# cloudflare/flow-pipeline

Measured on AMD Instinct MI355X. Metric: FlowMessages/sec aggregated into flows_5m, higher is better.
Workload: dtype u64

## Files before the change

flow-pipeline_amd/csrc/ingest.cuh:

```cuda
#pragma once
#include <hip/hip_runtime.h>
#include <stdint.h>

#include "sinks.cuh"

#ifndef FA_FOLD_EVERY
#define FA_FOLD_EVERY 4
#endif
#ifndef FA_LT_KEEP
#define FA_LT_KEEP 8u
#endif
namespace fa {

struct NoHook {
    __device__ __forceinline__ void operator()() const {}
};
struct LaneTally {
    uint32_t ok = 0, direct = 0, second = 0, misfit8 = 0, late = 0;
    uint32_t tick = 0;
};
template <int MODE, uint32_t KEYSETS, uint32_t COLS, bool T8 = false, int CANDM = -1, class Hook = NoHook>
__device__ __forceinline__ void lane_work(const KArgs& a, LdsTable<LDS_SLOTS>& lt, LdsMinutes& lm, uint32_t* part_cnt, const uint32_t* tile,
                                          bool mine, uint32_t pos, uint32_t end, uint32_t rec_idx, uint32_t tb_base,
                                          LaneTally& tally, uint32_t& pmode, uint32_t& lt_seen, uint32_t& lt_hits,
                                          uint4* bins, uint32_t* bin_cnt, uint32_t& fill_out, Hook&& after_parse = Hook(),
                                          CmsLds* cl = nullptr, uint32_t* cms_scratch = nullptr, HotAddrs* hot = nullptr,
                                          uint32_t* wpart_cnt = nullptr, uint32_t* seq = nullptr) {
    constexpr uint32_t TB = bin_cap<T8, bin_line(KEYSETS)>();
    bool sure = false, framed_ok = false;
    Rec r;
    rec_clear(r);
    if (mine) {
        LdsSrc src{tile};
        framed_ok = true;
        if (a.framed && !(FA_DBG(a, DBG_NO_FRAME))) {
            uint32_t pl = 0;
            const uint32_t i = pos >> 2;
            framed_ok = frame_short(fa_alignbyte(src.dw(i + 1), src.dw(i), pos), end - pos, pl);
            pos += pl;
        }
        sure = framed_ok && (FA_DBG(a, DBG_NO_PARSE)) != 0;
    }
    if (!FA_DBG(a, DBG_NO_PARSE)) {
        LdsAbsSrc src;
        const uint32_t tile_at = (uint32_t)(uintptr_t)(const __attribute__((address_space(3))) uint32_t*)tile;
        pos += tile_at;
        end += tile_at;
        const uint32_t n_mine = (uint32_t)__builtin_popcountll(__builtin_amdgcn_ballot_w64(framed_ok));
        auto most = [&](bool c) { return 2u * (uint32_t)__builtin_popcountll(__builtin_amdgcn_ballot_w64(c)) > n_mine; };
        if (pmode == 0u && !FA_DBG(a, DBG_LOOP_PARSER)) {
            if (framed_ok) sure = parse_tmpl<COLS, SHAPE_MOCKER>(src, pos, end, r);
        }
        bool need = framed_ok && !sure;
        if (pmode <= 1u && FA_ANY(need) && !FA_DBG(a, DBG_LOOP_PARSER | DBG_NO_SECOND)) {
            if (need) {
                rec_clear(r);
                sure = parse_tmpl<COLS, SHAPE_GOFLOW>(src, pos, end, r);
            }
            if (pmode < 1u && most(need && sure)) pmode = 1u;
        }
        need = framed_ok && !sure;
        if (pmode <= 2u && FA_ANY(need) && !FA_DBG(a, DBG_LOOP_PARSER | DBG_NO_SECOND)) {
            if (need) {
                rec_clear(r);
                sure = parse_canon<COLS, true>(src, pos, end, r);
            }
            if (pmode < 2u && most(need && sure)) pmode = 2u;
        }
        if (pmode == 4u && seq != nullptr && !FA_DBG(a, DBG_NO_SECOND)) {
            if (framed_ok) {
                sure = parse_seq<COLS>(src, pos, end, r, seq + 2, fa_uniform(seq[0]));
                if (!FA_DBG(a, DBG_LOOP_PARSER)) tally.second += sure ? 1u : 0u;
            }
        }
// ... 75 lines not shown
            if (vd && keys_on) pd = keyset_probe(a, a.ks_dst, dh1);
        }
    }
    if (ks_on<KEYSETS>(a, FA_KEYS_AS_PAIR)) {
        uint64_t k0 = 0, k1 = 0;
        const bool lt_on = lt_seen != 0xffffffffu && !(FA_DBG(a, DBG_NO_LDS_TABLE));
        uint32_t h = 0;
        if (!T8 || lt_on) {
            pack_key(tb, r.src_as, r.dst_as, r.etype, k0, k1);
            h = key_hash(k0, k1);
        }
        const uint64_t b = r.bytes, p = r.packets, c = 1;
        bool pending = sure;
        if (lt_on) {
            if (pending) pending = !lds_table_add<LDS_SLOTS, LDS_PROBES>(lt, k0, k1, h, b, p, c);
            lt_seen += (uint32_t)__builtin_popcountll(__builtin_amdgcn_ballot_w64(sure));
            lt_hits += (uint32_t)__builtin_popcountll(__builtin_amdgcn_ballot_w64(sure && !pending));
            if (lt_seen >= 256u) {
                if (lt_hits * FA_LT_KEEP < lt_seen) lt_seen = 0xffffffffu;
                else lt_seen = lt_hits = 0;
            }
        }
        uint32_t fill_part = 0xffffffffu;
        bool fits = false;
        uint32_t part = 0;
        uint4 tv = make_uint4(0, 0, 0, 0);
        if (pending && a.seg) {
            const uint32_t tbr = tb - tb_base;
            if (T8) {
                fits = t8_fits(r.src_as, r.dst_as, tbr, b, p, r.etype);
                const uint2 tc = t8_pack(r.src_as, r.dst_as, (uint32_t)b, (uint32_t)p, tbr, r.etype, tb_base, part);
                tv.x = tc.x;
                tv.y = tc.y;
                if (FA_ANY(!fits)) tally.misfit8 += (!fits && tup16_fits(tbr, b, p, r.etype)) ? 1u : 0u;
            } else {
                fits = tup16_fits(tbr, b, p, r.etype);
                part = h >> (32 - a.plog2);
                tv = tup16_pack(r.src_as, r.dst_as, (uint32_t)b, (uint32_t)p, tbr, r.etype);
            }
        }
        if (bins) {
            auto claim = [&]() {
                const uint32_t slot = __hip_atomic_fetch_add(&bin_cnt[part], 1u, __ATOMIC_ACQUIRE, __HIP_MEMORY_SCOPE_WORKGROUP) & 0xffffu;
                if (slot < TB) {
                    if (T8) reinterpret_cast<uint2*>(bins)[part * TB + slot] = make_uint2(tv.x, tv.y);
                    else bins[part * TB + slot] = tv;
                    __hip_atomic_fetch_add(&bin_cnt[part], 0x10000u, __ATOMIC_RELEASE, __HIP_MEMORY_SCOPE_WORKGROUP);
                    fill_part = slot == TB - 1 ? part : fill_part;
                    pending = false;
                }
            };
            if (pending && fits) {
                claim();
                if (pending) {
                    const uint32_t ob = lds_add_rtn_u32(&part_cnt[part], 0x10000u) >> 16;
                    if (ob < a.capb) {
                        const size_t at = (size_t)part * a.region + (size_t)blockIdx.x * a.capq + (a.capq - 1u - ob);
                        if (FA_DBG(a, DBG_TUPLE_LOCAL)) {
                            reinterpret_cast<uint2*>(a.seg)[(size_t)blockIdx.x * 512u + (at & 511u)] = make_uint2(tv.x, tv.y);
                        } else if (!(FA_DBG(a, DBG_NO_TUPLE_STORE | DBG_NO_SINGLES))) {
                            if (T8) reinterpret_cast<uint2*>(a.seg)[at] = make_uint2(tv.x, tv.y);
                            else a.seg[at] = tv;
                        }
                        pending = false;
                    } else {
                        lds_add_u32(&part_cnt[part], 0xffff0000u);
                    }
                }
            }
        }
        fill_out = fill_part;
        if (__builtin_amdgcn_ballot_w64(pending) != 0ull && !(FA_DBG(a, DBG_NO_GLOBAL))) {
            Slot* sp = nullptr;
            const KArgs ca = cold_args();
            if (pending) {
                tally.direct++;
                if (T8 && !lt_on) {
                    pack_key(tb, r.src_as, r.dst_as, r.etype, k0, k1);
                    h = key_hash(k0, k1);
                }
                sp = table_find_or_claim(ca, k0, k1, h);
                if (!sp) spill_park(ca, k0, k1, b, p, c);
            }
            quad_atomic_update(sp, b, p, c);
        }
    }
    if (KEYSETS & (FA_KEYS_SRCADDR_CMS | FA_KEYS_DSTADDR_CMS)) {
        if (!(FA_DBG(a, DBG_NO_CMS))) {
            if (cl && (CANDM >= 0 || a.cseg)) {
                uint32_t* list = const_cast<uint32_t*>(tile) + 256;
                if (on_s) cms_scatter(a, *cl, list, 0u, vs, ws, sh1, sh2);
                if (on_d) cms_scatter(a, *cl, list, 1u, vd, wd, dh1, dh2);
            } else {
                if (vs) cms_add(a.cms_src, a.cms_depth, a.cms_wl2, a.cms_seed, r.src, ws, a.cms_nrep);
                if (vd) cms_add(a.cms_dst, a.cms_depth, a.cms_wl2, a.cms_seed, r.dst, wd, a.cms_nrep);
            }
        }
        if (keys_on && !cand) keyset_finish2(a, vs, ps, sh1, slo, shi, vd, pd, dh1, dlo, dhi);
        if (keys_on && cand) {
            const bool is = vs && cand_pass(a.cand_src, a.cms_depth, a.cms_wl2, cms_key(sh1, sh2, a.cms_wl2), cw0s);
            const bool id = vd && cand_pass(a.cand_dst, a.cms_depth, a.cms_wl2, cms_key(dh1, dh2, a.cms_wl2), cw0d);
            if (FA_ANY(is || id) && !FA_DBG(a, DBG_CAND_NO_SET)) {
                if (is) keyset_insert_h(a, a.ks_src, slo, shi, sh1);
                if (id) keyset_insert_h(a, a.ks_dst, dlo, dhi, dh1);
            }
        }
// ... 204 lines not shown
            for (int i0 = 0; i0 < LDS_SLOTS; i0 += BLOCK) {
                const int i = i0 + tid;
                Slot* sp = nullptr;
                unsigned long long b = 0, p = 0, c = 0;
                if (i < LDS_SLOTS) {
                    const unsigned long long k0 = lt.k0[i], k1 = lt.k1[i];
                    b = lt.bytes[i];
                    p = lt.packets[i];
                    c = lt.count[i];
                    if (k0 != 0 && k1 != 0 && c != 0) {
                        sp = table_find_or_claim(a, k0, k1, key_hash(k0, k1));
                        if (!sp) spill_park(a, k0, k1, b, p, c);
                    }
                }
                quad_atomic_update(sp, b, p, c);
            }
        }
        block_counters_add(ctr_scratch, a.ctr, tally);
    }
}

template <bool ON>
struct CmsLdsOpt {
    CmsLds v;
    __device__ __forceinline__ CmsLds* get() { return &v; }
};
template <>
struct CmsLdsOpt<false> {
    __device__ __forceinline__ CmsLds* get() { return nullptr; }
};
template <uint32_t KEYSETS>
constexpr int wtile_block() { return wt_lean(KEYSETS) ? WBLOCK : WBLOCK_CMS; }
template <uint32_t KEYSETS>
constexpr int wtile_stride() { return wt_stride(KEYSETS); }
template <bool ON>
struct HotAddrsOpt {
    HotAddrs v;
    __device__ __forceinline__ HotAddrs* get() { return &v; }
};
template <>
struct HotAddrsOpt<false> {
    __device__ __forceinline__ HotAddrs* get() { return nullptr; }
};

template <uint32_t KEYSETS, bool T8, bool SEQ = false, int CANDM = -1>
__global__ __launch_bounds__(wtile_block<KEYSETS>(), wt_lean(KEYSETS) ? 6 : 4) void wtile_kernel(KArgs a) {
    constexpr uint32_t BL = bin_line(KEYSETS);
    constexpr uint32_t TB = bin_cap<T8, BL>();
    constexpr uint32_t COLS = cols_for_keysets<KEYSETS>();
    constexpr int WBLOCK = wtile_block<KEYSETS>();
    constexpr bool HAS_CMS = (KEYSETS & (FA_KEYS_SRCADDR_CMS | FA_KEYS_DSTADDR_CMS)) != 0;
    constexpr int WAVES = WBLOCK / 64;
    constexpr int WT_STRIDE = wtile_stride<KEYSETS>();
    __shared__ CmsLdsOpt<HAS_CMS> cms_lds;
    __shared__ HotAddrsOpt<HAS_CMS> hot_lds;
    __shared__ uint32_t cms_scratch_all[HAS_CMS ? WAVES * 16 : 1];
    __shared__ __attribute__((aligned(16))) uint32_t tiles[WAVES * WT_STRIDE / 4];
    __shared__ __attribute__((aligned(16))) uint4 bins[NPART_MAX * BL];
    __shared__ uint32_t bin_cnt[NPART_MAX];
    __shared__ uint32_t part_cnt[NPART_MAX];
    __shared__ uint32_t flush_scratch[WAVES * 16];
    constexpr bool HAS_APP = (KEYSETS & FA_KEYS_ADDR_PORT_PROTO) != 0;
    __shared__ uint32_t wpart_cnt[HAS_APP ? (1u << WIDE_PLOG2_MAX) + 2u : 1u];
    __shared__ LdsTable<LDS_SLOTS> lt;
    __shared__ LdsMinutes lm;
    constexpr bool HAS_SEQ = SEQ && KEYSETS == FA_KEYS_AS_PAIR;
    static_assert(!SEQ || KEYSETS == FA_KEYS_AS_PAIR, "the learnt-order variant exists for the flows_5m rollup alone");
    __shared__ uint32_t seq_all[HAS_SEQ ? WAVES * (SEQ_MAX + 2) : 1];

    const uint32_t tid = threadIdx.x, lane = tid & 63;
    const uint32_t wave = __builtin_amdgcn_readfirstlane(tid >> 6);
    if (HAS_SEQ && lane < 2) seq_all[wave * (SEQ_MAX + 2) + lane] = 0;
    if (KEYSETS & FA_KEYS_AS_PAIR) {
        lds_table_clear(lt);
        for (int i = tid; i < NPART_MAX; i += WBLOCK) {
            part_cnt[i] = 0;
            bin_cnt[i] = 0;
        }
    }
    if (KEYSETS & FA_KEYS_MINUTE_SERIES) lds_minutes_clear(lm);
    if (HAS_APP)
        for (int i = tid; i < (1 << WIDE_PLOG2_MAX) + 2; i += WBLOCK) wpart_cnt[i] = i < (1 << WIDE_PLOG2_MAX) ? 0u : 0xffffffffu;
    CmsLds* const cl = (HAS_CMS && (CANDM >= 0 || a.cseg)) ? cms_lds.get() : nullptr;
    HotAddrs* const hot = (HAS_CMS && (KEYSETS != KS_ALL || (a.key_sets & (FA_KEYS_SRCADDR_CMS | FA_KEYS_DSTADDR_CMS)))) ? hot_lds.get() : nullptr;
    if (HAS_CMS && cl)
        for (int i = tid; i < (int)(CMS_SETS * CMS_NPART); i += WBLOCK) {
            cl->bin_cnt[i] = 0;
            cl->part_cnt[i] = 0;
        }
    if (HAS_CMS && hot)
        for (int i = tid; i < (int)(CMS_SETS * HOT_SLOTS); i += WBLOCK) {
            const int set = i / HOT_SLOTS, sl = i % HOT_SLOTS;
            const size_t at = (size_t)blockIdx.x * (CMS_SETS * HOT_SLOTS) + i;
            const uint32_t tg = a.hot_seed_tag ? a.hot_seed_tag[at] : 0u;
            if (tg >= 2u) {
                const HotSeed sd = a.hot_seed[at];
                hot->lo[set][sl] = sd.lo;
                hot->hi[set][sl] = sd.hi;
                hot->w[set][sl] = 0;
            }
            hot->touched[set][sl] = 0;
            *hot->tag(set, sl) = tg >= 2u ? tg : 0u;
        }
    uint32_t* tile = tiles + wave * (WT_STRIDE / 4);

    LaneTally tally;
    uint32_t lt_seen = 0, lt_hits = 0, pmode = 0;
    uint32_t tb_base = 0;
    const uint32_t ntiles = (a.n + a.tile_recs - 1) / a.tile_recs;
    __shared__ uint32_t next_k;
    if (tid == 0) next_k = 2u * WAVES;
    const uint32_t wg_pos = (gridDim.x & 7u) == 0u ? (blockIdx.x & 7u) * (gridDim.x >> 3) + (blockIdx.x >> 3) : blockIdx.x;
    auto tile_after_next = [&]() {
        uint32_t k = 0;
        if (lane == 0) k = lds_add_rtn_u32(&next_k, 1u);
        return (uint32_t)__builtin_amdgcn_readfirstlane((int)k) * gridDim.x + wg_pos;
    };
    struct __attribute__((packed, aligned(4))) OffPair {
        uint32_t lo, hi;
    };
    struct Tile {
        uint32_t r0, nrec;
        uint32_t q0, q1;
    };
    auto tile_load = [&](uint32_t t) {
        Tile d{0, 0, 0, 0};
        if (t < ntiles) {
            d.r0 = t * a.tile_recs;
            d.nrec = min(a.tile_recs, a.n - d.r0);
            if (lane < d.nrec) {
                const OffPair v = *reinterpret_cast<const OffPair*>(a.off + d.r0 + lane);
                d.q0 = v.lo;
                d.q1 = v.hi;
            }
        }
        return d;
    };
    constexpr uint32_t CAP = (uint32_t)WT_STRIDE - 16u;
    auto issue_dma = [&](uint32_t lo, uint32_t hi) {
        const uint32_t cbase = lo & ~15u;
        const uint32_t nbytes = hi > cbase ? min(hi - cbase, CAP) : 0u;
        for (uint32_t o = lane * 16u; o < nbytes; o += 1024u)
            __builtin_amdgcn_global_load_lds((const __attribute__((address_space(1))) void*)(a.buf + cbase + o),
                                             (__attribute__((address_space(3))) void*)(tile + (o - lane * 16u) / 4u), 16, 0, 2);
    };
    Tile cur = tile_load(wave * gridDim.x + wg_pos);
    uint32_t cur_lo = (uint32_t)__builtin_amdgcn_readfirstlane((int)cur.q0);
    uint32_t cur_hi = cur.nrec ? min((uint32_t)__builtin_amdgcn_readlane((int)cur.q1, (int)(cur.nrec - 1u)), a.len) : 0u;
    bool live = lane < cur.nrec;
    __syncthreads();
    issue_dma(cur_lo, cur_hi);
    Tile nxt = tile_load((wave + WAVES) * gridDim.x + wg_pos);
    tb_base = probe_tb_base(a);
    if (blockIdx.x == 0 && tid == 0) a.ctr->tb_base = tb_base;
    uint32_t t2 = 0;
    bool t2_have = false;
    while (cur.nrec != 0) {
        dma_wait_all();
        if (!t2_have) {
            t2 = tile_after_next();
            t2_have = true;
        }
        const uint32_t cbase = cur_lo & ~15u;
        const bool valid = live && cur.q1 >= cur.q0 && cur.q0 >= cur_lo && cur.q1 <= cur_hi;
        const bool staged = valid && cur.q1 - cbase <= CAP;
        bool rest = valid && !staged;
        const bool hopeless = (live && !valid) || (rest && cur.q0 == cur_lo);
        if (FA_ANY(hopeless)) {
            if (hopeless) {
                unsigned int j = atomicAdd(&a.ctr->exotic_count[a.par], 1u);
                a.exotic_idx[j] = cur.r0 + lane;
            }
            rest = rest && !hopeless;
        }
        uint32_t fill = 0xffffffffu;
        lane_work<MODE_INGEST, KEYSETS, COLS, T8, CANDM>(a, lt, lm, part_cnt, tile, staged, cur.q0 - cbase, cur.q1 - cbase, cur.r0 + lane, tb_base, tally,
                                                  pmode, lt_seen, lt_hits, bins, bin_cnt, fill, NoHook(), cl, cms_scratch_all + (HAS_CMS ? wave * 16 : 0), hot,
                                                  (HAS_APP && a.wseg) ? wpart_cnt : nullptr, HAS_SEQ ? seq_all + wave * (SEQ_MAX + 2) : nullptr);
        if ((KEYSETS & FA_KEYS_AS_PAIR) && a.seg) bins_flush<T8, BL>(a, bins, bin_cnt, part_cnt, flush_scratch + wave * 16, fill, tb_base, tally.direct);
        const unsigned long long restm = __builtin_amdgcn_ballot_w64(rest);
        if (restm != 0ull) {
            live = rest;
            cur_lo = (uint32_t)__builtin_amdgcn_readlane((int)cur.q0, (int)__builtin_ctzll(restm));
            issue_dma(cur_lo, cur_hi);
            continue;
        }
        t2_have = false;
        cur = nxt;
        cur_lo = (uint32_t)__builtin_amdgcn_readfirstlane((int)cur.q0);
        cur_hi = cur.nrec ? min((uint32_t)__builtin_amdgcn_readlane((int)cur.q1, (int)(cur.nrec - 1u)), a.len) : 0u;
        live = lane < cur.nrec;
        issue_dma(cur_lo, cur_hi);
        nxt = tile_load(t2);
    }
    if ((KEYSETS & FA_KEYS_AS_PAIR) && a.seg) {
        __syncthreads();
        for (uint32_t idx = tid; idx < (uint32_t)NPART_MAX * TB; idx += WBLOCK) {
            const uint32_t p = idx / TB, sl = idx % TB;
            const uint32_t cnt = min(bin_cnt[p] & 0xffffu, TB);
            if (sl < cnt) {
                const uint32_t ob = (part_cnt[p] >> 16) + sl;
                uint4 tv = make_uint4(0, 0, 0, 0);
                uint2 tc = make_uint2(0, 0);
                if (T8) tc = reinterpret_cast<const uint2*>(bins)[idx];
                else tv = bins[idx];
                if (ob < a.capb) {
                    const size_t at = (size_t)p * a.region + (size_t)blockIdx.x * a.capq + (a.capq - 1u - ob);
                    if (!(FA_DBG(a, DBG_NO_TUPLE_STORE))) {
                        if (T8) reinterpret_cast<uint2*>(a.seg)[at] = tc;
                        else a.seg[at] = tv;
                    }
                } else {
                    TupleVals v;
                    if (T8) t8_unpack(tc, p, tb_base, v);
                    else tup16_unpack(tv, v);
                    uint64_t k0, k1;
                    pack_key(tb_base + v.tbr, v.src_as, v.dst_as, v.etype, k0, k1);
                    agg_global(cold_args(), k0, k1, key_hash(k0, k1), v.bytes, v.packets, 1);
                    tally.direct++;
                }
            }
        }
        __syncthreads();
        if (tid < NPART_MAX) {
            part_cnt[tid] += min(bin_cnt[tid] & 0xffffu, TB) << 16;
            bin_cnt[tid] = 0;
        }
        __syncthreads();
    }
    if (HAS_CMS && hot) {
        __syncthreads();
        for (int i = tid; i < (int)(CMS_SETS * HOT_SLOTS); i += WBLOCK) {
            const int set = i / HOT_SLOTS, sl = i % HOT_SLOTS;
            const uint32_t tg = *hot->tag(set, sl);
            const bool hit = tg >= 2u && hot->touched[set][sl] != 0;
            const unsigned long long lo = hot->lo[set][sl], hi = hot->hi[set][sl];
            if (hit) {
                const uint32_t key[4] = {(uint32_t)lo, (uint32_t)(lo >> 32), (uint32_t)hi, (uint32_t)(hi >> 32)};
                cms_add(set ? a.cms_dst : a.cms_src, a.cms_depth, a.cms_wl2, a.cms_seed, key, hot->w[set][sl], a.cms_nrep);
                if (!(FA_DBG(a, DBG_NO_KEYSET))) keyset_offer(a, (uint32_t)set, key);
            }
            if (a.hot_seed_tag) {
                const size_t at = (size_t)blockIdx.x * (CMS_SETS * HOT_SLOTS) + i;
                const unsigned long long wv = hit ? hot->w[set][sl] : ~0ull;
                unsigned long long wmin = wv;
                uint32_t nhit = hit ? 1u : 0u, amin = (uint32_t)sl;
// ... 204 lines not shown
```

flow-pipeline_amd/csrc/ingest_host.inc:

```

template <int MODE>
static int launch_tiles(fa_ctx* c, KArgs& a, int grid, fa_ctx::LaunchEvents* ev = nullptr) {
    dim3 b(BLOCK);
    dim3 g(grid);
    dim3 ge(std::min(256u, (a.n + BLOCK - 1) / BLOCK));
    a.par = c->par;
    c->par ^= 1u;
    const bool wave_tiles = MODE == MODE_INGEST && a.seg != nullptr && c->use_wave_tiles;
    const bool t8 = wave_tiles && c->use_t8;
    hipStream_t dstream = c->stream;
    if (ev) (void)hipEventRecord(ev->e0, c->stream);
    const bool seq_variant = wave_tiles && c->cfg.key_sets == FA_KEYS_AS_PAIR && c->seq_mode != 2 && (c->seq_mode == 1 || c->stats.batches < c->seq_until);
    if (seq_variant) c->stats.learnt_order_launches += 1;
    if (wave_tiles) c->stats.wave_tile_launches += 1;
    if (t8) c->stats.compact_tuple_launches += 1;
    if (MODE == MODE_INGEST && wave_tiles && a.wseg) HIPCHK(c, hipMemsetAsync(&c->d_ctr->wtb_min, 0xff, 2 * sizeof(unsigned int), c->stream));
#define FA_LAUNCH_W(KS)                                                                         \
    do {                                                                                        \
        if constexpr ((KS & 6u) != 0u && KS != KS_ALL) {   \
            if (a.cseg) {                                                      \
                if (c->cand_state) {                                                            \
                    if (t8) hipLaunchKernelGGL((wtile_kernel<KS, true, false, 1>), g, dim3(wtile_block<KS>()), 0, c->stream, a); \
                    else hipLaunchKernelGGL((wtile_kernel<KS, false, false, 1>), g, dim3(wtile_block<KS>()), 0, c->stream, a);   \
                } else {                                                                        \
// ... 420 lines not shown
        if (n > lim) {
            for (size_t i = 0; i < n; i += lim) {
                const size_t m = std::min(lim, n - i);
                int rc1 = ingest_device_records(c, d_buf, len, (size_t)((double)bytes * (double)m / (double)n), (const uint32_t*)d_off + i, m);
                if (rc1) return rc1;
            }
            return FA_OK;
        }
    }
    const bool scatter = (c->cfg.key_sets & FA_KEYS_AS_PAIR) && (c->sink_mode == 2 || (c->sink_mode == 0 && n >= (1u << 15)));
    c->use_wave_tiles = scatter;
    c->use_t8 = c->use_wave_tiles && c->plog2 == 8 && c->t8_mode != 2 && (c->t8_mode == 1 || c->stats.batches >= c->t8_wide_until);
    if (n > AGG_MAX_BATCH && !c->use_t8) {
        const size_t h = n / 2;
        int rc1 = ingest_device_records(c, d_buf, len, bytes / 2, d_off, h);
        if (rc1) return rc1;
        return ingest_device_records(c, d_buf, len, bytes - bytes / 2, (const uint32_t*)d_off + h, n - h);
    }
    int rc = pre_launch_guard(c, n);
    if (rc) return rc;
    rc = ensure_exotic(c, n);
    if (rc) return rc;
    if (c->ev_used == c->ev_pool.size()) {
        if (c->ev_pool.size() >= 4096) {
            rc = settle(c);
            if (rc) return rc;
        } else {
            fa_ctx::LaunchEvents e{};
            HIPCHK(c, hipEventCreate(&e.e0));
            HIPCHK(c, hipEventCreate(&e.e1));
            HIPCHK(c, hipEventCreate(&e.e2));
            c->ev_pool.push_back(e);
        }
    }
    KArgs a = make_args(c);
    a.buf = (const uint8_t*)d_buf;
    a.off = (const uint32_t*)d_off;
    a.n = (uint32_t)n;
    a.len = (uint32_t)len;
    a.tile_recs = tile_recs_for(bytes, n);
    int grid = tile_grid<MODE_INGEST>(c, a.n, a.tile_recs);
    if (c->use_wave_tiles) {
        const double avg = (double)bytes / (double)n;
        const bool big_wg = !wt_lean(c->cfg.key_sets);
        const uint32_t ks = c->cfg.key_sets;
        auto recs_for = [&](double cap) {
            double r = cap / avg;
            r = (cap - 2.0 * 12.0 * std::sqrt(std::min(r, (double)WT_RECS))) / avg;
            return r >= (double)WT_RECS ? (uint32_t)WT_RECS : r < 1.0 ? 1u : (uint32_t)r;
        };
        const double cap = (double)wt_stride((ks >= 1u && ks <= 7u) || ks == 9u ? ks : KS_ALL) - 16.0 - 15.0;
        a.tile_recs = recs_for(cap);
        const uint32_t wtiles = (a.n + a.tile_recs - 1) / a.tile_recs;
        const uint32_t waves = (uint32_t)(big_wg ? WBLOCK_CMS : WBLOCK) / 64u;
        const uint32_t wgs = (wtiles + waves - 1) / waves;
        grid = (int)std::max(1u, std::min<uint32_t>(wgs, (uint32_t)c->num_cus * (uint32_t)(big_wg ? 1 : WT_WG_PER_CU)));
    }
    if (scatter) {
        rc = ensure_segments(c, n, (uint32_t)grid, c->use_t8, a);
        if (rc) return rc;
    }
    if (c->use_wave_tiles && (c->cfg.key_sets & (FA_KEYS_SRCADDR_CMS | FA_KEYS_DSTADDR_CMS)) && !c->cms_atomic && c->cms_scatter_ok) {
        rc = ensure_csegments(c, n, (uint32_t)grid, a);
        if (rc) return rc;
    }
    if (c->use_wave_tiles && c->wtab && (c->cfg.key_sets & FA_KEYS_ADDR_PORT_PROTO) && grid <= WAGG_MAX_NWG &&
        (c->wide_mode == 2 || c->wide_mode == 3 || (c->wide_mode == 0 && c->wide_scatter))) {
        for (int guard = 0;; guard++) {
            rc = ensure_wsegments(c, n, (uint32_t)grid, a);
            if (rc) return rc;
            if (!table_args_stale(c, a)) break;
            if (guard >= 4) return fail(c, FA_ERR_HIP, "internal: tables keep moving while a launch is prepared");
            refresh_table_args(c, a);
        }
        c->wlog_now = c->wide_mode == 3 || (c->wide_mode == 0 && c->wide_defer);
    } else {
        c->wlog_now = false;
    }
    fa_ctx::LaunchEvents* evp = &c->ev_pool[c->ev_used++];
    if (c->wtab) c->wpot_total += (uint64_t)n * c->wide_per_record;
    rc = launch_tiles<MODE_INGEST>(c, a, grid, evp);
    if (rc) return rc;
    if (c->wlog_now && a.wseg) {
        rc = wlog_record(c, a, n);
        if (rc) return rc;
    } else if (c->wide_mode == 0 && !c->wide_defer && !c->wlog.empty()) {
        const fa_ctx::WChunk& k = c->wlog.front();
        if ((k.wplog2 == a.wplog2 && k.wmask == a.wmask) || c->stats.batches % 8 == 0) {
            rc = wlog_flush_oldest(c);
            if (rc) return rc;
        }
    }
    rc = post_launch_snapshot(c, n);
    if (rc) return rc;
    c->stats.bytes_in += bytes;
    c->stats.batches += 1;
    if (c->cfg.key_sets & (FA_KEYS_SRCADDR_CMS | FA_KEYS_DSTADDR_CMS)) {
        c->cms_dirty = c->cand_state == nullptr;
        c->merged_valid = false;
    }
    return FA_OK;
}

static constexpr size_t FRAME_DEVICE_MIN = (size_t)1 << 20;
static int frame_split_host(const uint8_t* buf, size_t len, std::vector<uint64_t>& off) {
    size_t p = 0;
    off.clear();
// ... 199 lines not shown
```

flow-pipeline_amd/csrc/sinks.cuh:

```cuda
#pragma once
#include <hip/hip_runtime.h>
#include <stdint.h>

#include "gen.cuh"
#include "table.cuh"
#include "wide.cuh"
#include "wire.cuh"

namespace fa {

constexpr int BLOCK = 256;
constexpr int TILE_BYTES = 21760;
constexpr int TILE_PAD = 112;
constexpr int TILE_STRIDE = TILE_BYTES + TILE_PAD;
constexpr int LDS_SLOTS = 64;
constexpr int LDS_PROBES = 2;
constexpr int PART_LOG2_MAX = 8;
constexpr int NPART_MAX = 1 << PART_LOG2_MAX;
#ifndef FA_WBLOCK
#define FA_WBLOCK 768
#endif
#ifndef FA_WT_STRIDE
#define FA_WT_STRIDE 4864
#endif
#ifndef FA_BIN_BYTES
#define FA_BIN_BYTES 64
#endif
constexpr int WBLOCK = FA_WBLOCK;
constexpr int WT_RECS = 64;
constexpr int WT_STRIDE = FA_WT_STRIDE;
constexpr int WT_STRIDE_CMS = 5056;
constexpr int WT_WG_PER_CU = 2;
constexpr int WBLOCK_CMS = 2 * FA_WBLOCK > 1024 ? 1024 : 2 * FA_WBLOCK;
static_assert(WBLOCK % 64 == 0 && WBLOCK >= 256 && WBLOCK <= 1024 && WT_STRIDE % 16 == 0, "wave-tile geometry");
static_assert(FA_BIN_BYTES == 128 || FA_BIN_BYTES == 64, "bin = one or half a cache line");
__host__ __device__ constexpr bool wt_lean(uint32_t key_sets) { return key_sets == FA_KEYS_AS_PAIR || key_sets == (FA_KEYS_AS_PAIR | FA_KEYS_ADDR_PORT_PROTO); }
__host__ __device__ constexpr int wt_stride(uint32_t key_sets) {
    return (wt_lean(key_sets) ? WT_STRIDE : WT_STRIDE_CMS) - ((key_sets & FA_KEYS_ADDR_PORT_PROTO) ? (wt_lean(key_sets) ? 128 : 160) : 0);
}
__host__ __device__ constexpr uint32_t bin_line(uint32_t key_sets) { return wt_lean(key_sets) ? FA_BIN_BYTES / 16u : 8u; }
template <bool T8, uint32_t BL>
constexpr uint32_t bin_cap() { return (T8 ? 2u : 1u) * BL; }
constexpr int AGG_BLOCK = 1024;
#ifndef FA_AGG_SLOTS
#define FA_AGG_SLOTS 4096
#endif
constexpr int AGG_SLOTS = FA_AGG_SLOTS;
constexpr int AGG_PROBES = 16;
constexpr uint32_t AGG_MAX_BATCH = 1u << 24;
constexpr uint32_t AGG8_MAX_BATCH = (1u << 25) - 1u;
static_assert(TILE_STRIDE % 16 == 0, "LDS tile buffers must stay 16-byte aligned");

enum { MODE_INGEST = 0, MODE_DECODE = 1 };
constexpr uint32_t KS_ALL = 0xFFu;
constexpr uint32_t FA_KEYS_WIDE = FA_KEYS_ADDR_PORT_PROTO | FA_KEYS_PORT_HIST | FA_KEYS_MINUTE_SERIES;
constexpr uint32_t PORT_DENSE = 65536;
#ifndef FA_ABLATE
#define FA_ABLATE 0
#endif
#ifndef FA_TL_WINDOW
#define FA_TL_WINDOW 256u
#endif
#define FA_DBG(a, flags) (FA_ABLATE != 0 && ((a).dbg & (flags)) != 0)
enum { DBG_NO_SINK = 1, DBG_LOOP_PARSER = 2, DBG_NO_LDS_TABLE = 4, DBG_NO_GLOBAL = 8, DBG_NO_PARSE = 16, DBG_NO_TUPLE_STORE = 32,
       DBG_AGG_NO_LDS = 64, DBG_AGG_NO_FLUSH = 128, DBG_AGG_NO_SLOW = 256, DBG_DMA_NO_NT = 512, DBG_TIMING = 1024, DBG_TUPLE_NT = 2048, DBG_TUPLE_SC = 4096, DBG_NO_LANE_OFF = 8192, DBG_SYNTH_TILES = 16384, DBG_NOT_MINE = 32768, DBG_NO_SECOND = 65536, DBG_NO_FRAME = 131072, DBG_NO_KEYSET = 262144, DBG_NO_CMS = 524288, DBG_NO_HOT = 1048576, DBG_CMS_TUPLE_LOCAL = 268435456 , DBG_NO_SINGLES = 134217728 , DBG_TUPLE_LOCAL = 67108864 , DBG_CAND_NO_SET = 33554432 , DBG_AGG_ATOMIC_FLUSH = 2097152 ,
       DBG_AGG8_TIMING = 8388608 ,
       DBG_CMS_TIMING = 4194304  };

struct SpillEntry {
    unsigned long long k0, k1, bytes, packets, count;
};

struct Counters {
    unsigned long long ok, bad, slow, spill_lost, used, direct, retried;
    unsigned long long misfit8;
    unsigned int exotic_count[2], retry_count[2];
    unsigned int spill_count, rows_count, ks_overflow, ks_rows;
    unsigned int tb_base, wtb_min, wtb_nmax, pad;
    unsigned long long t_wait, t_work, t_tiles, t_total;
    unsigned long long wfold_n;
    unsigned long long wused, wspill_lost;
    unsigned int wspill_count, wrows_count;
    unsigned long long agg_groups, agg_launches;
    unsigned long long late;
};

struct __attribute__((aligned(32))) KeySlot {
    unsigned long long tag, lo, hi, pad;
};
constexpr unsigned long long KS_CLAIMED = 1ull << 63, KS_READY = 1ull << 62;
struct TopkRow {
    unsigned long long lo, hi, weight;
};
// ... 727 lines not shown

template <bool T8, uint32_t BL>
__device__ __forceinline__ void bins_flush(const KArgs& a, uint4* bins, uint32_t* bin_cnt, uint32_t* part_cnt, uint32_t* scratch,
                                           uint32_t fill_part, uint32_t tb_base, uint32_t& n_direct) {
    constexpr uint32_t TB = bin_cap<T8, BL>();
    const unsigned long long fm = __builtin_amdgcn_ballot_w64(fill_part != 0xffffffffu);
    if (fm == 0ull) return;
    constexpr uint32_t LPB = BL, GROUPS = 64u / LPB;
    const uint32_t ln = __lane_id(), g = ln / LPB, sub = ln % LPB;
    const uint32_t rank = (uint32_t)__builtin_popcountll(fm & ((1ull << ln) - 1ull));
    const uint32_t todo = (uint32_t)__builtin_popcountll(fm);
    for (uint32_t base = 0; base < todo; base += GROUPS) {
        if (fill_part != 0xffffffffu && rank - base < GROUPS) scratch[rank - base] = fill_part;
        const bool act = g < min(GROUPS, todo - base);
        const uint32_t fp = act ? scratch[g] : 0u;
        const uint32_t c0 = __hip_atomic_load(&bin_cnt[fp], __ATOMIC_ACQUIRE, __HIP_MEMORY_SCOPE_WORKGROUP);
        const uint4 tq = bins[fp * BL + sub];
        uint32_t line = 0;
        if (act && sub == 0) line = atomicAdd(&part_cnt[fp], 1u) & 0xffffu;
        bool late = false;
        if (__builtin_amdgcn_ballot_w64(act && (c0 >> 16) < TB) != 0ull) {
            late = true;
            while (__builtin_amdgcn_ballot_w64(act && (__hip_atomic_load(&bin_cnt[fp], __ATOMIC_ACQUIRE, __HIP_MEMORY_SCOPE_WORKGROUP) >> 16) < TB) != 0ull) {}
        }
        line = (uint32_t)__shfl((int)line, (int)(ln - sub));
        if (act) {
            const uint4 tv = late ? bins[fp * BL + sub] : tq;
            if ((line + 1u) * TB <= a.capf) {
                const size_t seg0 = ((size_t)fp * a.region + (size_t)blockIdx.x * a.capq) >> (T8 ? 1 : 0);
                if (FA_DBG(a, DBG_TUPLE_LOCAL)) a.seg[(size_t)blockIdx.x * FA_TL_WINDOW + ((fp * (FA_TL_WINDOW > 256u ? 128u : 0u) + line * BL + sub) & (FA_TL_WINDOW - 1u))] = tv;
                else if (!(FA_DBG(a, DBG_NO_TUPLE_STORE))) a.seg[seg0 + line * BL + sub] = tv;
            } else {
                TupleVals v[2];
                if (T8) {
                    t8_unpack(make_uint2(tv.x, tv.y), fp, tb_base, v[0]);
                    t8_unpack(make_uint2(tv.z, tv.w), fp, tb_base, v[1]);
                } else {
                    tup16_unpack(tv, v[0]);
                }
#pragma unroll
                for (int e = 0; e < (T8 ? 2 : 1); e++) {
                    uint64_t q0, q1;
                    pack_key(tb_base + v[e].tbr, v[e].src_as, v[e].dst_as, v[e].etype, q0, q1);
                    agg_global(cold_args(), q0, q1, key_hash(q0, q1), v[e].bytes, v[e].packets, 1);
                    n_direct++;
                }
                if (sub == 0) atomicSub(&part_cnt[fp], 1u);
            }
            if (sub == 0) __hip_atomic_store(&bin_cnt[fp], 0u, __ATOMIC_RELEASE, __HIP_MEMORY_SCOPE_WORKGROUP);
        }
    }
}

}
```

Baseline: 47.31 billion.

## Dedicate drain waves to flush full bins and singles for AS-pair ingest

For the AS-pair-only keyset, the workgroup is split into parse waves and one or two drain waves. Parse waves publish full bins and overflow singles to LDS ring queues instead of flushing them to global memory inline. The drain wave streams those bins and singles to the global segments. The aim is to take global-store flush latency off the parse critical path, at the cost of one fewer parsing wave per workgroup, spin-wait polling, and extra LDS queue traffic.

Result: slower. 45.22 billion (-4.4%).

```diff
diff --git a/flow-pipeline_amd/csrc/ingest.cuh b/flow-pipeline_amd/csrc/ingest.cuh
--- a/flow-pipeline_amd/csrc/ingest.cuh
+++ b/flow-pipeline_amd/csrc/ingest.cuh
@@ -19,7 +19,7 @@
     uint32_t ok = 0, direct = 0, second = 0, misfit8 = 0, late = 0;
     uint32_t tick = 0;
 };
-template <int MODE, uint32_t KEYSETS, uint32_t COLS, bool T8 = false, int CANDM = -1, class Hook = NoHook>
+template <int MODE, uint32_t KEYSETS, uint32_t COLS, bool T8 = false, int CANDM = -1, int DRAIN = 0, class Hook = NoHook>
 __device__ __forceinline__ void lane_work(const KArgs& a, LdsTable<LDS_SLOTS>& lt, LdsMinutes& lm, uint32_t* part_cnt, const uint32_t* tile,
                                           bool mine, uint32_t pos, uint32_t end, uint32_t rec_idx, uint32_t tb_base,
                                           LaneTally& tally, uint32_t& pmode, uint32_t& lt_seen, uint32_t& lt_hits,
@@ -201,6 +201,10 @@
             };
             if (pending && fits) {
                 claim();
+                if constexpr (DRAIN > 0) {
+                    if (fill_part != 0xffffffffu) drain_publish_full(drain_lds<DRAIN, T8>.v[part % (uint32_t)DRAIN], part);
+                    if (pending && drain_offer_single(drain_lds<DRAIN, T8>.v[part % (uint32_t)DRAIN], part, tv)) pending = false;
+                }
                 if (pending) {
                     const uint32_t ob = lds_add_rtn_u32(&part_cnt[part], 0x10000u) >> 16;
                     if (ob < a.capb) {
@@ -511,10 +515,14 @@
     constexpr bool HAS_CMS = (KEYSETS & (FA_KEYS_SRCADDR_CMS | FA_KEYS_DSTADDR_CMS)) != 0;
     constexpr int WAVES = WBLOCK / 64;
     constexpr int WT_STRIDE = wtile_stride<KEYSETS>();
+    constexpr int NDRAIN = wt_drain_waves(KEYSETS);
+    constexpr int PWAVES = wt_parse_waves(KEYSETS);
+    static_assert(PWAVES + NDRAIN == WAVES && PWAVES >= 1, "waves of a workgroup");
+    static_assert(NDRAIN == 0 || sizeof(DrainState<T8>) <= (size_t)WT_STRIDE, "a drain wave's state fits the tile buffer it gave up");
     __shared__ CmsLdsOpt<HAS_CMS> cms_lds;
     __shared__ HotAddrsOpt<HAS_CMS> hot_lds;
     __shared__ uint32_t cms_scratch_all[HAS_CMS ? WAVES * 16 : 1];
-    __shared__ __attribute__((aligned(16))) uint32_t tiles[WAVES * WT_STRIDE / 4];
+    __shared__ __attribute__((aligned(16))) uint32_t tiles[PWAVES * WT_STRIDE / 4];
     __shared__ __attribute__((aligned(16))) uint4 bins[NPART_MAX * BL];
     __shared__ uint32_t bin_cnt[NPART_MAX];
     __shared__ uint32_t part_cnt[NPART_MAX];
@@ -525,11 +533,17 @@
     __shared__ LdsMinutes lm;
     constexpr bool HAS_SEQ = SEQ && KEYSETS == FA_KEYS_AS_PAIR;
     static_assert(!SEQ || KEYSETS == FA_KEYS_AS_PAIR, "the learnt-order variant exists for the flows_5m rollup alone");
-    __shared__ uint32_t seq_all[HAS_SEQ ? WAVES * (SEQ_MAX + 2) : 1];
+    __shared__ uint32_t seq_all[HAS_SEQ ? PWAVES * (SEQ_MAX + 2) : 1];
 
     const uint32_t tid = threadIdx.x, lane = tid & 63;
     const uint32_t wave = __builtin_amdgcn_readfirstlane(tid >> 6);
-    if (HAS_SEQ && lane < 2) seq_all[wave * (SEQ_MAX + 2) + lane] = 0;
+    bool drainer = false;
+    if constexpr (NDRAIN > 0) {
+        drainer = wave >= (uint32_t)PWAVES;
+        for (int d = 0; d < NDRAIN; d++) drain_state_clear(drain_lds<NDRAIN, T8>.v[d], tid, (uint32_t)WBLOCK);
+        if (tid == 0) drain_lds<NDRAIN, T8>.ndone = 0;
+    }
+    if (HAS_SEQ && lane < 2 && wave < (uint32_t)PWAVES) seq_all[wave * (SEQ_MAX + 2) + lane] = 0;
     if (KEYSETS & FA_KEYS_AS_PAIR) {
         lds_table_clear(lt);
         for (int i = tid; i < NPART_MAX; i += WBLOCK) {
@@ -568,7 +582,7 @@
     uint32_t tb_base = 0;
     const uint32_t ntiles = (a.n + a.tile_recs - 1) / a.tile_recs;
     __shared__ uint32_t next_k;
-    if (tid == 0) next_k = 2u * WAVES;
+    if (tid == 0) next_k = 2u * PWAVES;
     const uint32_t wg_pos = (gridDim.x & 7u) == 0u ? (blockIdx.x & 7u) * (gridDim.x >> 3) + (blockIdx.x >> 3) : blockIdx.x;
     auto tile_after_next = [&]() {
         uint32_t k = 0;
@@ -584,6 +598,9 @@
     };
     auto tile_load = [&](uint32_t t) {
         Tile d{0, 0, 0, 0};
+        if constexpr (NDRAIN > 0) {
+            if (drainer) return d;
+        }
         if (t < ntiles) {
             d.r0 = t * a.tile_recs;
             d.nrec = min(a.tile_recs, a.n - d.r0);
@@ -609,7 +626,7 @@
     bool live = lane < cur.nrec;
     __syncthreads();
     issue_dma(cur_lo, cur_hi);
-    Tile nxt = tile_load((wave + WAVES) * gridDim.x + wg_pos);
+    Tile nxt = tile_load((wave + PWAVES) * gridDim.x + wg_pos);
     tb_base = probe_tb_base(a);
     if (blockIdx.x == 0 && tid == 0) a.ctr->tb_base = tb_base;
     uint32_t t2 = 0;
@@ -633,10 +650,12 @@
             rest = rest && !hopeless;
         }
         uint32_t fill = 0xffffffffu;
-        lane_work<MODE_INGEST, KEYSETS, COLS, T8, CANDM>(a, lt, lm, part_cnt, tile, staged, cur.q0 - cbase, cur.q1 - cbase, cur.r0 + lane, tb_base, tally,
+        lane_work<MODE_INGEST, KEYSETS, COLS, T8, CANDM, NDRAIN>(a, lt, lm, part_cnt, tile, staged, cur.q0 - cbase, cur.q1 - cbase, cur.r0 + lane, tb_base, tally,
                                                   pmode, lt_seen, lt_hits, bins, bin_cnt, fill, NoHook(), cl, cms_scratch_all + (HAS_CMS ? wave * 16 : 0), hot,
                                                   (HAS_APP && a.wseg) ? wpart_cnt : nullptr, HAS_SEQ ? seq_all + wave * (SEQ_MAX + 2) : nullptr);
-        if ((KEYSETS & FA_KEYS_AS_PAIR) && a.seg) bins_flush<T8, BL>(a, bins, bin_cnt, part_cnt, flush_scratch + wave * 16, fill, tb_base, tally.direct);
+        if constexpr (NDRAIN == 0) {
+            if ((KEYSETS & FA_KEYS_AS_PAIR) && a.seg) bins_flush<T8, BL>(a, bins, bin_cnt, part_cnt, flush_scratch + wave * 16, fill, tb_base, tally.direct);
+        }
         const unsigned long long restm = __builtin_amdgcn_ballot_w64(rest);
         if (restm != 0ull) {
             live = rest;
@@ -651,6 +670,13 @@
         live = lane < cur.nrec;
         issue_dma(cur_lo, cur_hi);
         nxt = tile_load(t2);
+    }
+    if constexpr (NDRAIN > 0) {
+        if (drainer) {
+            drain_wave<T8, BL>(a, bins, bin_cnt, part_cnt, drain_lds<NDRAIN, T8>.v[wave - (uint32_t)PWAVES], &drain_lds<NDRAIN, T8>.ndone, (uint32_t)PWAVES, tb_base, tally.direct);
+        } else if (lane == 0) {
+            __hip_atomic_fetch_add(&drain_lds<NDRAIN, T8>.ndone, 1u, __ATOMIC_RELEASE, __HIP_MEMORY_SCOPE_WORKGROUP);
+        }
     }
     if ((KEYSETS & FA_KEYS_AS_PAIR) && a.seg) {
         __syncthreads();
diff --git a/flow-pipeline_amd/csrc/ingest_host.inc b/flow-pipeline_amd/csrc/ingest_host.inc
--- a/flow-pipeline_amd/csrc/ingest_host.inc
+++ b/flow-pipeline_amd/csrc/ingest_host.inc
@@ -496,7 +496,7 @@
         const double cap = (double)wt_stride((ks >= 1u && ks <= 7u) || ks == 9u ? ks : KS_ALL) - 16.0 - 15.0;
         a.tile_recs = recs_for(cap);
         const uint32_t wtiles = (a.n + a.tile_recs - 1) / a.tile_recs;
-        const uint32_t waves = (uint32_t)(big_wg ? WBLOCK_CMS : WBLOCK) / 64u;
+        const uint32_t waves = (uint32_t)wt_parse_waves(ks);
         const uint32_t wgs = (wtiles + waves - 1) / waves;
         grid = (int)std::max(1u, std::min<uint32_t>(wgs, (uint32_t)c->num_cus * (uint32_t)(big_wg ? 1 : WT_WG_PER_CU)));
     }
diff --git a/flow-pipeline_amd/csrc/sinks.cuh b/flow-pipeline_amd/csrc/sinks.cuh
--- a/flow-pipeline_amd/csrc/sinks.cuh
+++ b/flow-pipeline_amd/csrc/sinks.cuh
@@ -39,6 +39,12 @@
     return (wt_lean(key_sets) ? WT_STRIDE : WT_STRIDE_CMS) - ((key_sets & FA_KEYS_ADDR_PORT_PROTO) ? (wt_lean(key_sets) ? 128 : 160) : 0);
 }
 __host__ __device__ constexpr uint32_t bin_line(uint32_t key_sets) { return wt_lean(key_sets) ? FA_BIN_BYTES / 16u : 8u; }
+#ifndef FA_DRAIN_WAVES
+#define FA_DRAIN_WAVES 1
+#endif
+static_assert(FA_DRAIN_WAVES == 1 || FA_DRAIN_WAVES == 2, "drain waves of a lean workgroup");
+__host__ __device__ constexpr int wt_drain_waves(uint32_t key_sets) { return key_sets == FA_KEYS_AS_PAIR ? FA_DRAIN_WAVES : 0; }
+__host__ __device__ constexpr int wt_parse_waves(uint32_t key_sets) { return (wt_lean(key_sets) ? WBLOCK : WBLOCK_CMS) / 64 - wt_drain_waves(key_sets); }
 template <bool T8, uint32_t BL>
 constexpr uint32_t bin_cap() { return (T8 ? 2u : 1u) * BL; }
 constexpr int AGG_BLOCK = 1024;
@@ -872,4 +878,148 @@
     }
 }
 
-}
+template <bool T8>
+struct TupWord {
+    using type = uint4;
+};
+template <>
+struct TupWord<true> {
+    using type = uint2;
+};
+template <bool T8>
+struct __attribute__((aligned(16))) DrainState {
+    static constexpr uint32_t NS = T8 ? 256u : 128u;
+    typename TupWord<T8>::type stup[NS];
+    uint32_t spart[NS];
+    uint32_t full[NPART_MAX];
+    uint32_t ftail, stail;
+    int sfree;
+};
+template <int N, bool T8>
+struct DrainLds {
+    DrainState<T8> v[N];
+    uint32_t ndone;
+};
+template <int N, bool T8>
+__shared__ DrainLds<N, T8> drain_lds;
+template <bool T8>
+__device__ __forceinline__ void drain_state_clear(DrainState<T8>& ds, uint32_t tid, uint32_t nthreads) {
+    for (uint32_t i = tid; i < (uint32_t)NPART_MAX; i += nthreads) ds.full[i] = 0;
+    for (uint32_t i = tid; i < DrainState<T8>::NS; i += nthreads) ds.spart[i] = 0;
+    if (tid == 0) {
+        ds.ftail = 0;
+        ds.stail = 0;
+        ds.sfree = (int)DrainState<T8>::NS;
+    }
+}
+template <bool T8>
+__device__ __forceinline__ void drain_publish_full(DrainState<T8>& ds, uint32_t part) {
+    const uint32_t i = __hip_atomic_fetch_add(&ds.ftail, 1u, __ATOMIC_RELAXED, __HIP_MEMORY_SCOPE_WORKGROUP) & (uint32_t)(NPART_MAX - 1);
+    __hip_atomic_store(&ds.full[i], 0x80000000u | part, __ATOMIC_RELEASE, __HIP_MEMORY_SCOPE_WORKGROUP);
+}
+template <bool T8>
+__device__ __forceinline__ bool drain_offer_single(DrainState<T8>& ds, uint32_t part, const uint4& tv) {
+    if (__hip_atomic_fetch_sub(&ds.sfree, 1, __ATOMIC_ACQ_REL, __HIP_MEMORY_SCOPE_WORKGROUP) <= 0) {
+        __hip_atomic_fetch_add(&ds.sfree, 1, __ATOMIC_RELAXED, __HIP_MEMORY_SCOPE_WORKGROUP);
+        return false;
+    }
+    const uint32_t i = __hip_atomic_fetch_add(&ds.stail, 1u, __ATOMIC_ACQ_REL, __HIP_MEMORY_SCOPE_WORKGROUP) & (DrainState<T8>::NS - 1u);
+    if constexpr (T8) ds.stup[i] = make_uint2(tv.x, tv.y);
+    else ds.stup[i] = tv;
+    __hip_atomic_store(&ds.spart[i], 0x80000000u | part, __ATOMIC_RELEASE, __HIP_MEMORY_SCOPE_WORKGROUP);
+    return true;
+}
+template <bool T8, uint32_t BL>
+__device__ __forceinline__ void drain_wave(const KArgs& a, uint4* bins, uint32_t* bin_cnt, uint32_t* part_cnt, DrainState<T8>& ds,
+                                           uint32_t* ndone, uint32_t nparse, uint32_t tb_base, uint32_t& n_direct) {
+    constexpr uint32_t TB = bin_cap<T8, BL>();
+    constexpr uint32_t LPB = BL, GROUPS = 64u / LPB;
+    constexpr uint32_t NS = DrainState<T8>::NS;
+    const uint32_t ln = __lane_id(), g = ln / LPB, sub = ln % LPB;
+    uint32_t fhead = 0, shead = 0;
+    for (;;) {
+        const bool was_done = __hip_atomic_load(ndone, __ATOMIC_ACQUIRE, __HIP_MEMORY_SCOPE_WORKGROUP) == nparse;
+        uint32_t* const fent = &ds.full[(fhead + g) & (uint32_t)(NPART_MAX - 1)];
+        const uint32_t fe = __hip_atomic_load(fent, __ATOMIC_ACQUIRE, __HIP_MEMORY_SCOPE_WORKGROUP);
+        const unsigned long long finv = __builtin_amdgcn_ballot_w64(sub == 0 && (fe >> 31) == 0u);
+        const uint32_t nf = finv != 0ull ? (uint32_t)__builtin_ctzll(finv) / LPB : GROUPS;
+        if (nf != 0u) {
+            const bool act = g < nf;
+            const uint32_t fp = act ? ((uint32_t)__shfl((int)fe, (int)(ln - sub)) & 0xffffu) : 0u;
+            if (act && sub == 0) __hip_atomic_store(fent, 0u, __ATOMIC_RELAXED, __HIP_MEMORY_SCOPE_WORKGROUP);
+            const uint32_t c0 = __hip_atomic_load(&bin_cnt[fp], __ATOMIC_ACQUIRE, __HIP_MEMORY_SCOPE_WORKGROUP);
+            const uint4 tq = bins[fp * BL + sub];
+            uint32_t line = 0;
+            if (act && sub == 0) line = atomicAdd(&part_cnt[fp], 1u) & 0xffffu;
+            bool late = false;
+            if (__builtin_amdgcn_ballot_w64(act && (c0 >> 16) < TB) != 0ull) {
+                late = true;
+                while (__builtin_amdgcn_ballot_w64(act && (__hip_atomic_load(&bin_cnt[fp], __ATOMIC_ACQUIRE, __HIP_MEMORY_SCOPE_WORKGROUP) >> 16) < TB) != 0ull) {}
+            }
+            line = (uint32_t)__shfl((int)line, (int)(ln - sub));
+            if (act) {
+                const uint4 tv = late ? bins[fp * BL + sub] : tq;
+                if ((line + 1u) * TB <= a.capf) {
+                    const size_t seg0 = ((size_t)fp * a.region + (size_t)blockIdx.x * a.capq) >> (T8 ? 1 : 0);
+                    if (FA_DBG(a, DBG_TUPLE_LOCAL)) a.seg[(size_t)blockIdx.x * FA_TL_WINDOW + ((fp * (FA_TL_WINDOW > 256u ? 128u : 0u) + line * BL + sub) & (FA_TL_WINDOW - 1u))] = tv;
+                    else if (!(FA_DBG(a, DBG_NO_TUPLE_STORE))) a.seg[seg0 + line * BL + sub] = tv;
+                } else {
+                    TupleVals v[2];
+                    if (T8) {
+                        t8_unpack(make_uint2(tv.x, tv.y), fp, tb_base, v[0]);
+                        t8_unpack(make_uint2(tv.z, tv.w), fp, tb_base, v[1]);
+                    } else {
+                        tup16_unpack(tv, v[0]);
+                    }
+#pragma unroll
+                    for (int e = 0; e < (T8 ? 2 : 1); e++) {
+                        uint64_t q0, q1;
+                        pack_key(tb_base + v[e].tbr, v[e].src_as, v[e].dst_as, v[e].etype, q0, q1);
+                        agg_global(cold_args(), q0, q1, key_hash(q0, q1), v[e].bytes, v[e].packets, 1);
+                        n_direct++;
+                    }
+                    if (sub == 0) atomicSub(&part_cnt[fp], 1u);
+                }
+                if (sub == 0) __hip_atomic_store(&bin_cnt[fp], 0u, __ATOMIC_RELEASE, __HIP_MEMORY_SCOPE_WORKGROUP);
+            }
+            fhead += nf;
+        }
+        const uint32_t si = (shead + ln) & (NS - 1u);
+        const uint32_t se = __hip_atomic_load(&ds.spart[si], __ATOMIC_ACQUIRE, __HIP_MEMORY_SCOPE_WORKGROUP);
+        const unsigned long long sinv = __builtin_amdgcn_ballot_w64((se >> 31) == 0u);
+        const uint32_t ns = sinv != 0ull ? (uint32_t)__builtin_ctzll(sinv) : 64u;
+        if (ns != 0u) {
+            if (ln < ns) {
+                const typename TupWord<T8>::type tw = ds.stup[si];
+                __hip_atomic_store(&ds.spart[si], 0u, __ATOMIC_RELAXED, __HIP_MEMORY_SCOPE_WORKGROUP);
+                const uint32_t part = se & 0xffffu;
+                const uint32_t ob = lds_add_rtn_u32(&part_cnt[part], 0x10000u) >> 16;
+                if (ob < a.capb) {
+                    const size_t at = (size_t)part * a.region + (size_t)blockIdx.x * a.capq + (a.capq - 1u - ob);
+                    if (FA_DBG(a, DBG_TUPLE_LOCAL)) {
+                        reinterpret_cast<uint2*>(a.seg)[(size_t)blockIdx.x * 512u + (at & 511u)] = make_uint2(tw.x, tw.y);
+                    } else if (!(FA_DBG(a, DBG_NO_TUPLE_STORE | DBG_NO_SINGLES))) {
+                        reinterpret_cast<typename TupWord<T8>::type*>(a.seg)[at] = tw;
+                    }
+                } else {
+                    lds_add_u32(&part_cnt[part], 0xffff0000u);
+                    TupleVals v;
+                    if constexpr (T8) t8_unpack(tw, part, tb_base, v);
+                    else tup16_unpack(tw, v);
+                    uint64_t q0, q1;
+                    pack_key(tb_base + v.tbr, v.src_as, v.dst_as, v.etype, q0, q1);
+                    agg_global(cold_args(), q0, q1, key_hash(q0, q1), v.bytes, v.packets, 1);
+                    n_direct++;
+                }
+            }
+            shead += ns;
+            if (ln == 0) __hip_atomic_fetch_add(&ds.sfree, (int)ns, __ATOMIC_RELEASE, __HIP_MEMORY_SCOPE_WORKGROUP);
+        }
+        if (nf == 0u && ns == 0u) {
+            if (was_done) break;
+            __builtin_amdgcn_s_sleep(2);
+        }
+    }
+}
+
+}
```
